# baudm/parseq

Measured on NVIDIA H100. Metric: images/sec PARSeq-S 32x128 AR+1refine, higher is better.
Workload: dtype bf16

## Files before the change

### parseq_b200/build.py

```python
from __future__ import annotations

import os
import shutil
import subprocess

PKG = os.path.dirname(os.path.abspath(__file__))
CSRC = os.path.join(PKG, "csrc")
LIB_DIR = os.path.join(PKG, "lib")
LIB_PATH = os.path.join(LIB_DIR, "libparseq_b200.so")
SOURCES = ["engine.cu"]
HEADERS = ["ptx.cuh", "gemm.cuh", "kernels.cuh", "dec_ar.cuh", "dec_ar2.cuh", "gemm_ln.cuh", "mlp_ln.cuh", "attn_wgmma.cuh", "qkv_attn.cuh", "crops.cuh", os.path.join("..", "..", "include", "parseq_b200.h")]

NVCC_FLAGS = [
    "-gencode", "arch=compute_90a,code=sm_90a", "-lineinfo", "-O3", "-std=c++17",
    "-Xcompiler", "-fPIC", "-shared",
]


def _nvcc() -> str:
    for cand in (os.environ.get("NVCC"), shutil.which("nvcc"), "/usr/local/cuda/bin/nvcc"):
        if cand and os.path.exists(cand):
            return cand
    raise RuntimeError("nvcc not found")


def needs_build() -> bool:
    if not os.path.exists(LIB_PATH):
        return True
    t = os.path.getmtime(LIB_PATH)
    deps = [os.path.join(CSRC, s) for s in SOURCES + HEADERS]
    return any(os.path.getmtime(d) > t for d in deps)


def build(force: bool = False, verbose: bool = False) -> str:
    if not force and not needs_build():
        return LIB_PATH
    import fcntl
    os.makedirs(LIB_DIR, exist_ok=True)
    with open(os.path.join(LIB_DIR, ".build.lock"), "w") as lock:
        fcntl.flock(lock, fcntl.LOCK_EX)
        if not force and not needs_build():
            return LIB_PATH
        tmp = LIB_PATH + f".tmp{os.getpid()}"
        cmd = [_nvcc()] + NVCC_FLAGS + ["-o", tmp] + [os.path.join(CSRC, s) for s in SOURCES]
        if verbose:
            cmd.insert(1, "-Xptxas=-v")
        res = subprocess.run(cmd, capture_output=True, text=True)
        if res.returncode != 0:
            if os.path.exists(tmp):
                os.remove(tmp)
            raise RuntimeError("nvcc failed:\n" + res.stdout + res.stderr)
        os.replace(tmp, LIB_PATH)
        if verbose:
            print(res.stderr)
    return LIB_PATH


if __name__ == "__main__":
    print(build(force=True, verbose=True))
```

### parseq_b200/csrc/engine.cu

```cuda
#include <cuda.h>
#include <cuda_runtime.h>

#include <cmath>
#include <cstdio>
#include <cstdlib>
#include <cstring>
#include <map>
#include <mutex>
#include <set>
#include <string>
#include <type_traits>
#include <vector>

#include "../../include/parseq_b200.h"
#include "gemm.cuh"
#include "kernels.cuh"
#include "dec_ar.cuh"
#include "dec_ar2.cuh"
#include "gemm_ln.cuh"
#include "mlp_ln.cuh"
#include "attn_wgmma.cuh"
#include "qkv_attn.cuh"
#include "crops.cuh"

namespace {

constexpr int kMaxHeadClasses = 16384;
constexpr int kMaxLabelLength = 63;

thread_local std::string g_last_error;

int fail(int code, const std::string& msg) {
  g_last_error = msg;
  return code;
}
#define PQ_CUDA(expr)                                                                              \
  do {                                                                                             \
    cudaError_t _e = (expr);                                                                       \
    if (_e != cudaSuccess)                                                                         \
      return fail(PARSEQ_ERR_CUDA, std::string(#expr) + " -> " + cudaGetErrorString(_e));          \
  } while (0)
#define PQ_TRY(expr)                 \
  do {                               \
    int _r = (expr);                 \
    if (_r != PARSEQ_OK) return _r;  \
  } while (0)

typedef CUresult (*PFN_encodeTiled)(CUtensorMap*, CUtensorMapDataType, cuuint32_t, void*, const cuuint64_t*,
                                    const cuuint64_t*, const cuuint32_t*, const cuuint32_t*, CUtensorMapInterleave,
                                    CUtensorMapSwizzle, CUtensorMapL2promotion, CUtensorMapFloatOOBfill);
PFN_encodeTiled g_encode = nullptr;

int load_driver_api() {
  if (g_encode != nullptr) return PARSEQ_OK;
  void* fn = nullptr;
  cudaDriverEntryPointQueryResult qres;
  cudaError_t e = cudaGetDriverEntryPoint("cuTensorMapEncodeTiled", &fn, cudaEnableDefault, &qres);
  if (e != cudaSuccess || fn == nullptr || qres != cudaDriverEntryPointSuccess)
    return fail(PARSEQ_ERR_CUDA, "cuTensorMapEncodeTiled not available from the driver");
  g_encode = reinterpret_cast<PFN_encodeTiled>(fn);
  return PARSEQ_OK;
}

int make_tmap(CUtensorMap* tm, const void* ptr, int esize, long long rows, long long cols, long long ld, int box_cols,
              int box_rows) {
  PQ_TRY(load_driver_api());
  if ((reinterpret_cast<uintptr_t>(ptr) & 15u) != 0 || ((ld * esize) & 15) != 0)
    return fail(PARSEQ_ERR_INVALID_ARG, "GEMM operand must be 16-byte aligned with a 16-byte multiple row stride");
  cuuint64_t dims[2] = {static_cast<cuuint64_t>(cols), static_cast<cuuint64_t>(rows)};
  cuuint64_t strides[1] = {static_cast<cuuint64_t>(ld) * static_cast<cuuint64_t>(esize)};
  cuuint32_t box[2] = {static_cast<cuuint32_t>(box_cols), static_cast<cuuint32_t>(box_rows)};
  cuuint32_t estr[2] = {1, 1};
  CUresult r = g_encode(tm, esize == 2 ? CU_TENSOR_MAP_DATA_TYPE_BFLOAT16 : CU_TENSOR_MAP_DATA_TYPE_FLOAT32, 2,
// ... 4 lines not shown
  return PARSEQ_OK;
}

int make_tmap3d(CUtensorMap* tm, const void* ptr, long long d0, long long d1, long long d2, long long ld1, long long ld2,
                int box_d0, int box_d1) {
  PQ_TRY(load_driver_api());
  if ((reinterpret_cast<uintptr_t>(ptr) & 15u) != 0 || ((ld1 * 2) & 15) != 0 || ((ld2 * 2) & 15) != 0)
    return fail(PARSEQ_ERR_INVALID_ARG, "tensor map operand must be 16-byte aligned with 16-byte multiple strides");
  cuuint64_t dims[3] = {static_cast<cuuint64_t>(d0), static_cast<cuuint64_t>(d1), static_cast<cuuint64_t>(d2)};
  cuuint64_t strides[2] = {static_cast<cuuint64_t>(ld1) * 2u, static_cast<cuuint64_t>(ld2) * 2u};
  cuuint32_t box[3] = {static_cast<cuuint32_t>(box_d0), static_cast<cuuint32_t>(box_d1), 1u};
  cuuint32_t estr[3] = {1, 1, 1};
  CUresult r = g_encode(tm, CU_TENSOR_MAP_DATA_TYPE_BFLOAT16, 3, const_cast<void*>(ptr), dims, strides, box, estr,
                        CU_TENSOR_MAP_INTERLEAVE_NONE, CU_TENSOR_MAP_SWIZZLE_128B, CU_TENSOR_MAP_L2_PROMOTION_L2_256B,
                        CU_TENSOR_MAP_FLOAT_OOB_FILL_NONE);
  if (r != CUDA_SUCCESS) return fail(PARSEQ_ERR_CUDA, "cuTensorMapEncodeTiled(3d) failed: " + std::to_string(int(r)));
  return PARSEQ_OK;
}

int make_tmap_kv4d(CUtensorMap* tm, const void* ptr, int T, int max_batch, int panels, int box_t) {
  PQ_TRY(load_driver_api());
  if ((reinterpret_cast<uintptr_t>(ptr) & 15u) != 0)
    return fail(PARSEQ_ERR_INVALID_ARG, "tensor map operand must be 16-byte aligned");
  const cuuint64_t row = 128;
  cuuint64_t dims[4] = {64, static_cast<cuuint64_t>(T), static_cast<cuuint64_t>(max_batch), static_cast<cuuint64_t>(panels)};
  cuuint64_t strides[3] = {row, row * T, row * T * max_batch};
  cuuint32_t box[4] = {64, static_cast<cuuint32_t>(box_t), 1u, 1u};
  cuuint32_t estr[4] = {1, 1, 1, 1};
  CUresult r = g_encode(tm, CU_TENSOR_MAP_DATA_TYPE_BFLOAT16, 4, const_cast<void*>(ptr), dims, strides, box, estr,
                        CU_TENSOR_MAP_INTERLEAVE_NONE, CU_TENSOR_MAP_SWIZZLE_128B, CU_TENSOR_MAP_L2_PROMOTION_L2_256B,
                        CU_TENSOR_MAP_FLOAT_OOB_FILL_NONE);
  if (r != CUDA_SUCCESS) return fail(PARSEQ_ERR_CUDA, "cuTensorMapEncodeTiled(K/V 4d) failed: " + std::to_string(int(r)));
  return PARSEQ_OK;
}

uint16_t f32_to_bf16_rne(float f) {
  uint32_t u;
  std::memcpy(&u, &f, 4);
  if ((u & 0x7fffffffu) > 0x7f800000u) return static_cast<uint16_t>((u >> 16) | 0x40u);
  u += 0x7fffu + ((u >> 16) & 1u);
  return static_cast<uint16_t>(u >> 16);
}

struct LaunchOpts {
  int sm_count = 0;
  bool use_pdl = true;
  int ln_cta_group = 0;
  int ln_split = 0;
  int mlp_cta_group = 0;
  bool pair_pdl = false;
  int gemm_stages = 0;
  int attn_impl = 0;
  int ln_clusters = 0;
};
LaunchOpts g_default_opts;

int ensure_sm_count(LaunchOpts& o) {
  if (o.sm_count == 0) {
    int dev = 0;
    PQ_CUDA(cudaGetDevice(&dev));
    PQ_CUDA(cudaDeviceGetAttribute(&o.sm_count, cudaDevAttrMultiProcessorCount, dev));
  }
  return PARSEQ_OK;
}

struct LaunchConfig {
  cudaLaunchConfig_t cfg{};
  cudaLaunchAttribute attr[2];
  LaunchConfig(dim3 grid, dim3 block, size_t smem, cudaStream_t st, unsigned cluster, bool pdl) {
    cfg.gridDim = grid;
    cfg.blockDim = block;
    cfg.dynamicSmemBytes = smem;
    cfg.stream = st;
    cfg.attrs = attr;
    if (cluster > 0) {
      attr[cfg.numAttrs].id = cudaLaunchAttributeClusterDimension;
      attr[cfg.numAttrs].val.clusterDim.x = cluster;
      attr[cfg.numAttrs].val.clusterDim.y = 1;
      attr[cfg.numAttrs].val.clusterDim.z = 1;
      ++cfg.numAttrs;
    }
    if (pdl) {
      attr[cfg.numAttrs].id = cudaLaunchAttributeProgrammaticStreamSerialization;
      attr[cfg.numAttrs].val.programmaticStreamSerializationAllowed = 1;
      ++cfg.numAttrs;
    }
  }
  LaunchConfig(const LaunchConfig&) = delete;
  LaunchConfig& operator=(const LaunchConfig&) = delete;
};

template <typename... KArgs, typename... Args>
int launch_ex(const LaunchConfig& lc, void (*kern)(KArgs...), Args... args) {
  PQ_CUDA(cudaLaunchKernelEx(&lc.cfg, kern, static_cast<KArgs>(args)...));
  return PARSEQ_OK;
}
template <typename... KArgs, typename... Args>
int launch_k(const LaunchOpts& lo, void (*kern)(KArgs...), dim3 grid, dim3 block, size_t smem, cudaStream_t st, Args... args) {
  return launch_ex(LaunchConfig(grid, block, smem, st, 0, lo.use_pdl), kern, args...);
}
bool cluster_pdl(const LaunchOpts& lo, int cg) { return lo.use_pdl && (cg == 1 || lo.pair_pdl); }

template <typename F>
int dispatch_width(int D, const char* what, F&& f) {
  switch (D) {
    case 192: return f(std::integral_constant<int, 192>{});
// ... 42 lines not shown
    else return pq::dec_ar2_kernel<D, MT, CS, HS>;
  }
}
template <typename... KArgs>
int set_smem(void (*kern)(KArgs...), size_t bytes) {
  PQ_CUDA(cudaFuncSetAttribute(kern, cudaFuncAttributeMaxDynamicSharedMemorySize, static_cast<int>(bytes)));
  return PARSEQ_OK;
}
template <int D, int MT, int CS, bool WIDE, int IDP>
int ar2_attr() {
  PQ_TRY(set_smem(ar2_kernel<D, MT, CS, false, WIDE, IDP>(), pq::dec_ar2_smem_bytes<D, MT, CS, IDP>()));
  if constexpr (MT == 1 && CS == 8 && D / 64 <= CS)
    PQ_TRY(set_smem(ar2_kernel<D, MT, CS, true, WIDE, IDP>(), pq::dec_ar2_smem_bytes<D, MT, CS, IDP>()));
  return PARSEQ_OK;
}
template <bool WIDE, int IDP>
int ar2_set_attributes() {
  PQ_TRY((ar2_attr<192, 1, 8, WIDE, IDP>())); PQ_TRY((ar2_attr<192, 2, 8, WIDE, IDP>())); PQ_TRY((ar2_attr<384, 1, 8, WIDE, IDP>()));
  PQ_TRY((ar2_attr<384, 2, 8, WIDE, IDP>())); PQ_TRY((ar2_attr<768, 1, 8, WIDE, IDP>()));
  PQ_TRY((ar2_attr<192, 1, 6, WIDE, IDP>())); PQ_TRY((ar2_attr<192, 2, 6, WIDE, IDP>())); PQ_TRY((ar2_attr<384, 1, 6, WIDE, IDP>()));
  PQ_TRY((ar2_attr<384, 2, 6, WIDE, IDP>())); PQ_TRY((ar2_attr<768, 1, 6, WIDE, IDP>()));
  return PARSEQ_OK;
}

template <int D, int MODE>
int gemm_ln_attr() { return set_smem(pq::gemm_ln_fused_kernel<D, MODE>, pq::GemmLnCfg<D, MODE>::kSmemBytes); }
template <int D, int CG>
int mlp_ln_attr() { return set_smem(pq::mlp_ln_fused_kernel<D, CG>, pq::MlpLnCfg<D, CG>::kSmemBytes); }
template <int NK>
int attn_wgmma_attr() { return set_smem(pq::enc_attention_wgmma_kernel<NK>, pq::atw_smem_bytes<NK>()); }
template <int D>
int qkv_attn_attr() { return set_smem(pq::enc_qkv_attn_kernel<D>, pq::QkvAttnCfg::kSmemBytes); }
template <int EPI, int STORE>
int gemm_attr() { return set_smem(pq::gemm_bf16_wgmma_kernel<EPI, STORE>, pq::GemmCfg::smem_bytes<STORE != pq::ST_REG>()); }
constexpr int kTmaBenchSmem = 12 * pq::A2_SLOT + 1024 + 256;

int init_kernel_attributes() {
  PQ_TRY(set_smem(pq::dec_ar_kernel<192, 1>, pq::dec_ar_smem_bytes<192>()));
  PQ_TRY(set_smem(pq::dec_ar_kernel<192, 2>, pq::dec_ar_smem_bytes<192>()));
  PQ_TRY(set_smem(pq::dec_ar_kernel<384, 1>, pq::dec_ar_smem_bytes<384>()));
  PQ_TRY(set_smem(pq::dec_ar_kernel<384, 2>, pq::dec_ar_smem_bytes<384>()));
  PQ_TRY(set_smem(pq::dec_ar_kernel<768, 1>, pq::dec_ar_smem_bytes<768>()));
  PQ_TRY(set_smem(pq::dec_ar_kernel<768, 2>, pq::dec_ar_smem_bytes<768>()));
  PQ_TRY((ar2_set_attributes<false, 32>()));
  PQ_TRY((ar2_set_attributes<true, 32>()));
  PQ_TRY((ar2_set_attributes<false, 64>()));
  PQ_TRY((ar2_set_attributes<true, 64>()));
  PQ_TRY(set_smem(pq::dec_ln_head_argmax_kernel<192>, 120 * 1024));
  PQ_TRY(set_smem(pq::dec_ln_head_argmax_kernel<384>, 160 * 1024));
  PQ_TRY(set_smem(pq::dec_ln_head_argmax_kernel<768>, 226 * 1024));
  PQ_TRY((gemm_ln_attr<192, 0>())); PQ_TRY((gemm_ln_attr<384, 0>())); PQ_TRY((gemm_ln_attr<192, 1>()));
  PQ_TRY((gemm_ln_attr<384, 1>())); PQ_TRY((gemm_ln_attr<384, 2>()));
  PQ_TRY((mlp_ln_attr<192, 1>())); PQ_TRY((mlp_ln_attr<384, 1>())); PQ_TRY((mlp_ln_attr<192, 2>())); PQ_TRY((mlp_ln_attr<384, 2>()));
  PQ_TRY((attn_wgmma_attr<128>())); PQ_TRY((attn_wgmma_attr<256>()));
  PQ_TRY((qkv_attn_attr<192>())); PQ_TRY((qkv_attn_attr<384>()));
  PQ_TRY((gemm_attr<pq::EPI_F32, pq::ST_REG>()));
  PQ_TRY((gemm_attr<pq::EPI_F32_RESID, pq::ST_REG>()));
  PQ_TRY((gemm_attr<pq::EPI_BF16, pq::ST_REG>()));
  PQ_TRY((gemm_attr<pq::EPI_BF16, pq::ST_TMA_2D>()));
  PQ_TRY((gemm_attr<pq::EPI_BF16, pq::ST_TMA_3D>()));
  PQ_TRY((gemm_attr<pq::EPI_GELU_BF16, pq::ST_REG>()));
  PQ_TRY((gemm_attr<pq::EPI_GELU_BF16, pq::ST_TMA_2D>()));
  PQ_TRY(set_smem(pq::tma_stream_bench_kernel, kTmaBenchSmem));
  int dev = 0, optin = 0;
  PQ_CUDA(cudaGetDevice(&dev));
  PQ_CUDA(cudaDeviceGetAttribute(&optin, cudaDevAttrMaxSharedMemoryPerBlockOptin, dev));
  PQ_TRY(set_smem(pq::crop_resize_bicubic_kernel, static_cast<size_t>(optin)));
  return PARSEQ_OK;
}

int ensure_kernel_attributes() {
  static std::mutex mu;
  static std::set<int> done;
  int dev = 0;
  PQ_CUDA(cudaGetDevice(&dev));
  std::lock_guard<std::mutex> lock(mu);
  if (done.count(dev) != 0) return PARSEQ_OK;
  PQ_TRY(init_kernel_attributes());
  done.insert(dev);
  return PARSEQ_OK;
}

int gemm_launch(LaunchOpts& lo, const void* A, long long lda, const void* W, long long ldw, const float* bias, int M, int N,
                int K, int mode, float alpha, const float* resid, long long ldr, int resid_mod, void* out, long long ldo,
                cudaStream_t st, long long blocked_rows = 0) {
  if (M <= 0 || N <= 0 || K <= 0) return fail(PARSEQ_ERR_INVALID_ARG, "gemm: empty problem");
  if (mode != pq::EPI_F32 && mode != pq::EPI_BF16 && mode != pq::EPI_GELU_BF16)
    return fail(PARSEQ_ERR_INVALID_ARG, "gemm: mode must be 0 (fp32), 1 (bf16) or 2 (GELU bf16)");
  PQ_TRY(ensure_sm_count(lo));
  CUtensorMap ta, tb, to;
  PQ_TRY(make_tmap(&ta, A, 2, M, K, lda, pq::GEMM_BLOCK_K, pq::GEMM_BLOCK_M));
  PQ_TRY(make_tmap(&tb, W, 2, N, K, ldw, pq::GEMM_BLOCK_K, pq::GEMM_BLOCK_N));
  pq::GemmParams p;
  p.M = M; p.N = N; p.K = K; p.alpha = alpha; p.bias = bias;
  p.resid = resid; p.ldr = ldr; p.resid_mod = resid_mod; p.out = out; p.ldo = ldo;
  const int esz = (mode == pq::EPI_F32) ? 4 : 2;
  bool vec = ((reinterpret_cast<uintptr_t>(out) & 7u) == 0) && ((ldo * esz) % 8 == 0);
  if (resid != nullptr) vec = vec && ((reinterpret_cast<uintptr_t>(resid) & 7u) == 0) && ((ldr * 4) % 8 == 0);
  p.vec_ok = vec ? 1 : 0;
  int store = pq::ST_REG;
  if (blocked_rows > 0) {
    if (mode != pq::EPI_BF16 || N % 64 != 0 || blocked_rows < M || (reinterpret_cast<uintptr_t>(out) & 15u) != 0)
      return fail(PARSEQ_ERR_INVALID_ARG, "gemm: blocked output needs a bf16 epilogue, N % 64 == 0 and rows >= M");
    PQ_TRY(make_tmap3d(&to, out, 64, M, N / 64, 64, 64 * blocked_rows, 64, pq::GEMM_BLOCK_M));
    store = pq::ST_TMA_3D;
  } else if (mode != pq::EPI_F32 && (reinterpret_cast<uintptr_t>(out) & 15u) == 0 && (ldo * 2) % 16 == 0 && ldo >= N) {
// ... 31 lines not shown
  pq::GemmLnParams p;
  p.M = M; p.K = K; p.bias = bias; p.gamma = gamma; p.beta = beta; p.eps = eps;
  p.num_m_tiles = (M + Cfg::kTileM - 1) / Cfg::kTileM;
  int clusters = p.num_m_tiles;
  if constexpr (MODE == 2) {
    PQ_TRY(make_tmap(&tx, x, 4, M, D, D, Cfg::kXBoxCols, pq::GLN_BLOCK_M));
    if (lo.ln_clusters == 0) {
      const LaunchConfig occ(dim3(static_cast<unsigned>(lo.sm_count / Cfg::kCG * Cfg::kCG)), dim3(pq::GLN_THREADS),
                             Cfg::kSmemBytes, st, Cfg::kCG, false);
      PQ_CUDA(cudaOccupancyMaxActiveClusters(&lo.ln_clusters, pq::gemm_ln_fused_kernel<D, MODE>, &occ.cfg));
      if (lo.ln_clusters <= 0) return fail(PARSEQ_ERR_CUDA, "gemm_ln: no cluster of the persistent kernel fits the device");
    }
    clusters = std::min(p.num_m_tiles, lo.ln_clusters);
  } else {
    tx = ta;
  }
  return launch_ex(LaunchConfig(dim3(static_cast<unsigned>(clusters * Cfg::kCG)), dim3(pq::GLN_THREADS), Cfg::kSmemBytes, st,
                                Cfg::kCG, cluster_pdl(lo, Cfg::kCG)),
                   pq::gemm_ln_fused_kernel<D, MODE>, ta, tb, tx, x, reinterpret_cast<__nv_bfloat16*>(xn), p);
}
int gemm_ln_launch(LaunchOpts& lo, const void* A, long long lda, const void* W, long long ldw, const float* bias, int M, int D,
                   int K, float* x, const float* gamma, const float* beta, float eps, void* xn, cudaStream_t st) {
  if (M <= 0 || K <= 0) return fail(PARSEQ_ERR_INVALID_ARG, "gemm_ln: empty problem");
  PQ_TRY(ensure_sm_count(lo));
  PQ_TRY(load_driver_api());
  if (D == 384 && lo.ln_split != 1)
    return launch_gemm_ln<384, 2>(lo, A, lda, W, ldw, bias, M, K, x, gamma, beta, eps, xn, st);
  if (lo.ln_cta_group == 2) {
    if (D == 384) return launch_gemm_ln<384, 1>(lo, A, lda, W, ldw, bias, M, K, x, gamma, beta, eps, xn, st);
    if (D == 192) return launch_gemm_ln<192, 1>(lo, A, lda, W, ldw, bias, M, K, x, gamma, beta, eps, xn, st);
  }
  if (D == 384) return launch_gemm_ln<384, 0>(lo, A, lda, W, ldw, bias, M, K, x, gamma, beta, eps, xn, st);
  if (D == 192) return launch_gemm_ln<192, 0>(lo, A, lda, W, ldw, bias, M, K, x, gamma, beta, eps, xn, st);
  return fail(PARSEQ_ERR_UNSUPPORTED, "gemm_ln: embed_dim must be 192 or 384");
}

template <int D, int CG>
int launch_mlp_ln(const LaunchOpts& lo, const void* xn, const void* W1, const float* b1, const void* W2, const float* b2, int M,
                  float* x, const float* gamma, const float* beta, float eps, void* xn_out, cudaStream_t st) {
  using Cfg = pq::MlpLnCfg<D, CG>;
  if ((reinterpret_cast<uintptr_t>(x) & 7u) != 0 || (reinterpret_cast<uintptr_t>(xn_out) & 3u) != 0)
    return fail(PARSEQ_ERR_INVALID_ARG, "mlp_ln: x must be 8-byte and xn_out 4-byte aligned");
  CUtensorMap txn, tw1, tw2;
  PQ_TRY(make_tmap(&txn, xn, 2, M, D, D, 64, pq::GLN_BLOCK_M));
  PQ_TRY(make_tmap(&tw1, W1, 2, Cfg::kH, D, D, 64, Cfg::kW1Rows));
  PQ_TRY(make_tmap(&tw2, W2, 2, D, Cfg::kH, Cfg::kH, 64, Cfg::kW2Rows));
  pq::MlpLnParams p;
  p.M = M; p.b1 = b1; p.b2 = b2; p.gamma = gamma; p.beta = beta; p.eps = eps;
  p.num_m_tiles = (M + pq::GLN_BLOCK_M * CG - 1) / (pq::GLN_BLOCK_M * CG);
  return launch_ex(LaunchConfig(dim3(static_cast<unsigned>(p.num_m_tiles * CG)), dim3(pq::MLP_THREADS), Cfg::kSmemBytes, st, CG,
                                cluster_pdl(lo, CG)),
                   pq::mlp_ln_fused_kernel<D, CG>, txn, tw1, tw2, x, reinterpret_cast<__nv_bfloat16*>(xn_out), p);
}
int mlp_ln_launch(LaunchOpts& lo, const void* xn, const void* W1, const float* b1, const void* W2, const float* b2, int M, int D,
                  float* x, const float* gamma, const float* beta, float eps, void* xn_out, cudaStream_t st) {
  if (M <= 0) return fail(PARSEQ_ERR_INVALID_ARG, "mlp_ln: empty problem");
  PQ_TRY(ensure_sm_count(lo));
  PQ_TRY(load_driver_api());
  const int CG = lo.mlp_cta_group ? lo.mlp_cta_group : 2;
  if (CG == 2) {
    if (D == 384) return launch_mlp_ln<384, 2>(lo, xn, W1, b1, W2, b2, M, x, gamma, beta, eps, xn_out, st);
    if (D == 192) return launch_mlp_ln<192, 2>(lo, xn, W1, b1, W2, b2, M, x, gamma, beta, eps, xn_out, st);
  }
  if (D == 384) return launch_mlp_ln<384, 1>(lo, xn, W1, b1, W2, b2, M, x, gamma, beta, eps, xn_out, st);
  if (D == 192) return launch_mlp_ln<192, 1>(lo, xn, W1, b1, W2, b2, M, x, gamma, beta, eps, xn_out, st);
  return fail(PARSEQ_ERR_UNSUPPORTED, "mlp_ln: embed_dim must be 192 or 384 (hidden width 4 * embed_dim)");
}

int layernorm_launch(const LaunchOpts& lo, const float* x, const float* g, const float* b, float eps, int M, int D, void* y, float* y32,
                     cudaStream_t st, const float* add = nullptr, int add_mod = 1, float* xw = nullptr) {
  const int rows_per_block = 8;
  const int grid = (M + rows_per_block - 1) / rows_per_block;
  __nv_bfloat16* yb = reinterpret_cast<__nv_bfloat16*>(y);
  switch (D) {
    case 192: return launch_k(lo, pq::layernorm_kernel<192>, dim3(grid), dim3(256), 0, st, x, g, b, eps, M, yb, y32, add, add_mod, xw);
    case 384: return launch_k(lo, pq::layernorm_kernel<384>, dim3(grid), dim3(256), 0, st, x, g, b, eps, M, yb, y32, add, add_mod, xw);
    case 768: return launch_k(lo, pq::layernorm_kernel<768>, dim3(grid), dim3(256), 0, st, x, g, b, eps, M, yb, y32, add, add_mod, xw);
    default: return fail(PARSEQ_ERR_UNSUPPORTED, "layernorm: embed_dim must be 192, 384 or 768");
  }
}

int enc_attention_launch(const LaunchOpts& lo, const void* qkv, int B, int T, int D, int heads, void* out, cudaStream_t st) {
  if (D != heads * pq::ATT_DH) return fail(PARSEQ_ERR_UNSUPPORTED, "encoder attention kernels cover head_dim=64");
  if (lo.attn_impl == 1 && T <= 256) {
    const dim3 grid(static_cast<unsigned>(B * heads), static_cast<unsigned>((T + 127) / 128));
    const __nv_bfloat16* q = reinterpret_cast<const __nv_bfloat16*>(qkv);
    __nv_bfloat16* o = reinterpret_cast<__nv_bfloat16*>(out);
    if (T <= 128)
      return launch_k(lo, pq::enc_attention_wgmma_kernel<128>, grid, dim3(pq::ATW_THREADS), pq::atw_smem_bytes<128>(), st, q, o, T, D, heads);
    return launch_k(lo, pq::enc_attention_wgmma_kernel<256>, grid, dim3(pq::ATW_THREADS), pq::atw_smem_bytes<256>(), st, q, o, T, D, heads);
  }
  if (T != pq::ATT_T) {
    return launch_k(lo, pq::enc_attention_any_kernel, dim3(B * heads, (T + pq::ATT_T - 1) / pq::ATT_T), dim3(256), 0, st,
                    reinterpret_cast<const __nv_bfloat16*>(qkv), reinterpret_cast<__nv_bfloat16*>(out), T, D, heads);
  }
  return launch_k(lo, pq::enc_attention_kernel, dim3(B * heads), dim3(256), 0, st,
                  reinterpret_cast<const __nv_bfloat16*>(qkv), reinterpret_cast<__nv_bfloat16*>(out), D, heads);
}

bool qkv_attn_supported(int T, int D, int heads) { return T == pq::ATT_T && D == heads * pq::ATT_DH && (D == 192 || D == 384); }
int qkv_attn_launch(LaunchOpts& lo, const void* xn, const void* W, const float* bias, int B, int T, int D, int heads, void* out,
                    cudaStream_t st) {
  if (B <= 0) return fail(PARSEQ_ERR_INVALID_ARG, "qkv_attn: empty batch");
  if (!qkv_attn_supported(T, D, heads))
    return fail(PARSEQ_ERR_UNSUPPORTED, "qkv_attn: T = 128, head_dim 64 and embed_dim 192 or 384 only");
  if ((reinterpret_cast<uintptr_t>(out) & 15u) != 0) return fail(PARSEQ_ERR_INVALID_ARG, "qkv_attn: out must be 16-byte aligned");
  PQ_TRY(ensure_sm_count(lo));
  CUtensorMap tx, tw;
  PQ_TRY(make_tmap(&tx, xn, 2, static_cast<long long>(B) * T, D, D, pq::GEMM_BLOCK_K, pq::ATT_T));
  PQ_TRY(make_tmap(&tw, W, 2, 3 * D, D, D, pq::GEMM_BLOCK_K, pq::ATT_DH));
  const int items = B * heads;
// ... 1484 lines not shown
  const int D = e->D;
  const int cap = e->dec_chunk * e->L;
  parseq_engine::Stage& sg = e->stages[0];
  for (int r0 = 0; r0 < rows; r0 += cap) {
    const int n = (rows - r0 < cap) ? (rows - r0) : cap;
    const long long n4 = 1ll * n * D / 4;
    pq::f32_to_bf16_kernel<<<static_cast<unsigned>(std::min<long long>((n4 + 255) / 256, 132ll * 8)), 256, 0, e->main>>>(
        reinterpret_cast<const float4*>(x + 1ll * r0 * D), reinterpret_cast<uint2*>(sg.yn), n4);
    PQ_CUDA(cudaGetLastError());
    e->launches++;
    e->cur_cat = CAT_DEC_GEMM;
    PQ_TRY(gemm(e, sg.yn, D, e->w("head.weight"), D, e->wf("head.bias"), n, e->C, D, pq::EPI_F32, 1.0f, nullptr, 0, 0,
                logits + 1ll * r0 * e->C, e->C, e->main));
  }
  PQ_CUDA(cudaEventRecord(e->ev_out, e->main));
  PQ_CUDA(cudaStreamWaitEvent(user, e->ev_out, 0));
  return PARSEQ_OK;
}

int parseq_text_embed(parseq_engine* e, int32_t n, const int32_t* ids, float* out, parseq_stream_t stream) {
  if (e == nullptr || ids == nullptr || out == nullptr) return fail(PARSEQ_ERR_INVALID_ARG, "null argument");
  if (e->arch != 0) return fail(PARSEQ_ERR_UNSUPPORTED, "text_embed: PARSeq only");
  if (n <= 0) return n == 0 ? PARSEQ_OK : fail(PARSEQ_ERR_INVALID_ARG, "negative count");
  if (!e->slots[e->index.at("text_embed.embedding.weight")].set) return fail(PARSEQ_ERR_STATE, "weights not set");
  PQ_CUDA(cudaSetDevice(e->cfg.device));
  const long long total = 1ll * n * e->D;
  pq::text_embed_kernel<<<static_cast<unsigned>(std::min<long long>((total + 255) / 256, 132ll * 8)), 256, 0,
                          reinterpret_cast<cudaStream_t>(stream)>>>(ids, e->wf("text_embed.embedding.weight"), out, n, e->D, e->V,
                                                                    std::sqrt(static_cast<float>(e->D)));
  PQ_CUDA(cudaGetLastError());
  return PARSEQ_OK;
}

int parseq_bench_tma_stream(void* buf, int64_t bytes, int cluster, int ctas, int nboxes, int nslot, int mode, void* sink,
                            parseq_stream_t stream) {
  if (buf == nullptr || sink == nullptr || cluster < 1 || cluster > 8 || ctas % cluster != 0 || nslot < 1 || nslot > 12)
    return fail(PARSEQ_ERR_INVALID_ARG, "bench_tma_stream: bad arguments");
  const long long rows_total = 8192;
  const int blocks = static_cast<int>(bytes / (rows_total * 128));
  if (blocks < 1) return fail(PARSEQ_ERR_INVALID_ARG, "bench_tma_stream: buffer too small");
  PQ_TRY(ensure_kernel_attributes());
  CUtensorMap map;
  PQ_TRY(make_tmap3d(&map, buf, 64, rows_total, blocks, 64, 64 * rows_total, 64, 128));
  return launch_ex(LaunchConfig(dim3(static_cast<unsigned>(ctas)), dim3(pq::A2_THREADS + 32), kTmaBenchSmem,
                                reinterpret_cast<cudaStream_t>(stream), cluster > 1 ? static_cast<unsigned>(cluster) : 0, false),
                   pq::tma_stream_bench_kernel, map, nboxes, nslot, static_cast<int>(rows_total / 128), blocks, mode,
                   static_cast<unsigned int*>(sink));
}

int64_t parseq_debug_int(parseq_engine* e, const char* name) {
  if (name == nullptr) return -1;
  const std::string n(name);
  if (n == "ln_clusters") return (e ? e->lo : g_default_opts).ln_clusters;
  if (e == nullptr) return -1;
  if (n == "ar2_occupancy_mt1_cs8") return e->ar2_occ[1][0];
  if (n == "ar2_occupancy_mt2_cs8") return e->ar2_occ[2][0];
  if (n == "ar2_occupancy_mt1_cs6") return e->ar2_occ[1][1];
  if (n == "ar2_occupancy_mt2_cs6") return e->ar2_occ[2][1];
  if (n == "ar_last_cluster_size") return e->ar_last_cs;
  if (n == "ar_last_per") return e->ar_last_per;
  if (n == "ar_last_clusters") return e->ar_last_ncl;
  if (n == "ar_last_mt") return e->ar_last_mt;
  if (n == "ar_last_head_split") return e->ar_last_hs;
  if (n == "ar_last_wide") return e->ar_last_wide;
  if (n == "ar_last_ids_pitch") return e->ar_last_idp;
  if (n == "sm_count") return e->lo.sm_count;
  return -1;
}
int64_t parseq_kernel_launches(const parseq_engine* e) { return e ? e->launches : 0; }

int parseq_set_option(parseq_engine* e, const char* name, int64_t value) {
  if (name == nullptr) return fail(PARSEQ_ERR_INVALID_ARG, "null option");
  const std::string n(name);
  LaunchOpts& lo = e ? e->lo : g_default_opts;
  if (n == "block_n") {
    if (value != 0 && value != 64 && value != 128 && value != 192 && value != 256)
      return fail(PARSEQ_ERR_INVALID_ARG, "block_n: 0/64/128/192/256");
    return PARSEQ_OK;
  }
  if (n == "cta_group") {
    if (value < 0 || value > 2) return fail(PARSEQ_ERR_INVALID_ARG, "cta_group: 0 (auto) / 1 / 2");
    return PARSEQ_OK;
  }
  if (n == "attn_impl") { lo.attn_impl = value != 0 ? 1 : 0; if (e) drop_graphs(e); return PARSEQ_OK; }
  if (n == "pdl") { lo.use_pdl = value != 0; if (e) drop_graphs(e); return PARSEQ_OK; }
  if (n == "gemm_stages") {
    if (value < 0 || value == 1) return fail(PARSEQ_ERR_INVALID_ARG, "gemm_stages: 0 (full ring) or >= 2");
    lo.gemm_stages = static_cast<int>(value);
    if (e) drop_graphs(e);
    return PARSEQ_OK;
  }
  if (n == "ln_cta_group") {
    if (value < 0 || value > 2) return fail(PARSEQ_ERR_INVALID_ARG, "ln_cta_group: 0 (auto) / 1 / 2");
    lo.ln_cta_group = static_cast<int>(value);
    if (e) drop_graphs(e);
    return PARSEQ_OK;
  }
  if (n == "ln_split") {
    if (value < 0 || value > 2) return fail(PARSEQ_ERR_INVALID_ARG, "ln_split: 0 (auto) / 1 (off) / 2 (on)");
    lo.ln_split = static_cast<int>(value);
    if (e) drop_graphs(e);
    return PARSEQ_OK;
  }
  if (n == "mlp_cta_group") {
    if (value < 0 || value > 2) return fail(PARSEQ_ERR_INVALID_ARG, "mlp_cta_group: 0 (auto) / 1 / 2");
    lo.mlp_cta_group = static_cast<int>(value);
// ... 134 lines not shown
```

### parseq_b200/csrc/ptx.cuh

```cuda
#pragma once
#include <cuda_bf16.h>
#include <cuda_runtime.h>
#include <stdint.h>

namespace pq {

__device__ __forceinline__ uint32_t smem_u32(const void* p) {
  return static_cast<uint32_t>(__cvta_generic_to_shared(p));
}
__device__ __forceinline__ uint32_t lane_id() { return threadIdx.x & 31u; }

constexpr int ARGMAX_NONE = 0x7fffffff;
__device__ __forceinline__ bool argmax_better(float v, int j, float best, int bi) {
  if (j == ARGMAX_NONE) return false;
  if (bi == ARGMAX_NONE) return true;
  const bool vn = isnan(v), bn = isnan(best);
  if (vn != bn) return vn;
  if (vn || v == best) return j < bi;
  return v > best;
}
__device__ __forceinline__ void argmax_fold(float& best, int& bi, float v, int j) {
  if (argmax_better(v, j, best, bi)) { best = v; bi = j; }
}
__device__ __forceinline__ void argmax_shfl(float& best, int& bi, int lo = 1, int hi = 32) {
// ... 103 lines not shown
__device__ __forceinline__ void prefetch_tmap(const void* tmap) {
  asm volatile("prefetch.tensormap [%0];" ::"l"(reinterpret_cast<uint64_t>(tmap)) : "memory");
}
__device__ __forceinline__ void tma_load_2d(void* smem_dst, const void* tmap, uint64_t* bar, int32_t c0,
                                            int32_t c1) {
  asm volatile(
      "cp.async.bulk.tensor.2d.shared::cluster.global.mbarrier::complete_tx::bytes [%0], [%1, {%3, %4}], [%2];"
      ::"r"(smem_u32(smem_dst)), "l"(reinterpret_cast<uint64_t>(tmap)), "r"(smem_u32(bar)), "r"(c0), "r"(c1)
      : "memory");
}

__device__ __forceinline__ void tma_load_3d(void* smem_dst, const void* tmap, uint64_t* bar, int32_t c0, int32_t c1,
                                            int32_t c2) {
  asm volatile(
      "cp.async.bulk.tensor.3d.shared::cluster.global.mbarrier::complete_tx::bytes [%0], [%1, {%3, %4, %5}], [%2];"
      ::"r"(smem_u32(smem_dst)), "l"(reinterpret_cast<uint64_t>(tmap)), "r"(smem_u32(bar)), "r"(c0), "r"(c1), "r"(c2)
      : "memory");
}

__device__ __forceinline__ void tma_load_4d(void* smem_dst, const void* tmap, uint64_t* bar, int32_t c0, int32_t c1,
                                            int32_t c2, int32_t c3) {
  asm volatile(
      "cp.async.bulk.tensor.4d.shared::cluster.global.mbarrier::complete_tx::bytes [%0], [%1, {%3, %4, %5, %6}], [%2];"
      ::"r"(smem_u32(smem_dst)), "l"(reinterpret_cast<uint64_t>(tmap)), "r"(smem_u32(bar)), "r"(c0), "r"(c1), "r"(c2),
        "r"(c3)
      : "memory");
}

__device__ __forceinline__ void tma_store_2d(const void* tmap, const void* smem_src, int32_t c0, int32_t c1) {
  asm volatile("cp.async.bulk.tensor.2d.global.shared::cta.bulk_group [%0, {%2, %3}], [%1];"
               ::"l"(reinterpret_cast<uint64_t>(tmap)), "r"(smem_u32(smem_src)), "r"(c0), "r"(c1)
               : "memory");
}
__device__ __forceinline__ void tma_store_3d(const void* tmap, const void* smem_src, int32_t c0, int32_t c1, int32_t c2) {
  asm volatile("cp.async.bulk.tensor.3d.global.shared::cta.bulk_group [%0, {%2, %3, %4}], [%1];"
               ::"l"(reinterpret_cast<uint64_t>(tmap)), "r"(smem_u32(smem_src)), "r"(c0), "r"(c1), "r"(c2)
               : "memory");
}
__device__ __forceinline__ void tma_reduce_add_2d(const void* tmap, const void* smem_src, int32_t c0, int32_t c1) {
  asm volatile("cp.reduce.async.bulk.tensor.2d.global.shared::cta.add.tile.bulk_group [%0, {%2, %3}], [%1];"
               ::"l"(reinterpret_cast<uint64_t>(tmap)), "r"(smem_u32(smem_src)), "r"(c0), "r"(c1)
               : "memory");
}
__device__ __forceinline__ void bulk_commit_group() { asm volatile("cp.async.bulk.commit_group;" ::: "memory"); }
template <int N>
__device__ __forceinline__ void bulk_wait_group_read() {
  asm volatile("cp.async.bulk.wait_group.read %0;" ::"n"(N) : "memory");
}
template <int N>
__device__ __forceinline__ void bulk_wait_group() {
  asm volatile("cp.async.bulk.wait_group %0;" ::"n"(N) : "memory");
}
__device__ __forceinline__ void fence_proxy_async_smem() { asm volatile("fence.proxy.async.shared::cta;" ::: "memory"); }

__device__ __forceinline__ void tma_load_2d_mcast(void* smem_dst, const void* tmap, uint64_t* bar, int32_t c0, int32_t c1,
                                                  uint16_t cta_mask) {
  asm volatile(
      "cp.async.bulk.tensor.2d.shared::cluster.global.mbarrier::complete_tx::bytes.multicast::cluster [%0], [%1, {%3, %4}], [%2], %5;"
      ::"r"(smem_u32(smem_dst)), "l"(reinterpret_cast<uint64_t>(tmap)), "r"(smem_u32(bar)), "r"(c0), "r"(c1), "h"(cta_mask)
      : "memory");
}
__device__ __forceinline__ void mbar_wait_cluster(uint64_t* bar, uint32_t parity) {
  uint32_t ok = 0;
  long long t0 = clock64();
  uint32_t it = 0;
  while (true) {
    asm volatile(
        "{\n\t.reg .pred p;\n\t"
        "mbarrier.try_wait.parity.acquire.cluster.shared::cta.b64 p, [%1], %2;\n\t"
        "selp.b32 %0, 1, 0, p;\n\t}"
        : "=r"(ok)
        : "r"(smem_u32(bar)), "r"(parity)
        : "memory");
    if (ok) return;
    if (((++it) & 0x3ffu) == 0 && (clock64() - t0) > PQ_SPIN_LIMIT_CYCLES) __trap();
  }
}
__device__ __forceinline__ void st_cluster_f32(uint32_t cluster_addr, float v) {
  asm volatile("st.shared::cluster.f32 [%0], %1;" ::"r"(cluster_addr), "f"(v) : "memory");
}

__device__ __forceinline__ uint64_t make_desc_k_sw128(uint32_t smem_addr) {
  uint64_t d = 0;
  d |= static_cast<uint64_t>((smem_addr >> 4) & 0x3FFFu);
  d |= static_cast<uint64_t>(1u) << 16;
  d |= static_cast<uint64_t>(1024u >> 4) << 32;
  d |= static_cast<uint64_t>(1u) << 62;
  return d;
}
__device__ __forceinline__ void wgmma_fence() { asm volatile("wgmma.fence.sync.aligned;" ::: "memory"); }
__device__ __forceinline__ void wgmma_commit() { asm volatile("wgmma.commit_group.sync.aligned;" ::: "memory"); }
template <int N>
__device__ __forceinline__ void wgmma_wait() { asm volatile("wgmma.wait_group.sync.aligned %0;" ::"n"(N) : "memory"); }
template <int R>
__device__ __forceinline__ void wgmma_reg_fence(float (&d)[R]) {
#pragma unroll
  for (int i = 0; i < R; ++i) asm volatile("" : "+f"(d[i])::"memory");
}

template <int N>
__device__ __forceinline__ void wgmma_bf16(float (&d)[N / 2], uint64_t da, uint64_t db, uint32_t accumulate);
template <>
__device__ __forceinline__ void wgmma_bf16<32>(float (&d)[16], uint64_t da, uint64_t db, uint32_t accumulate) {
  asm volatile(
      "{\n\t.reg .pred p;\n\tsetp.ne.b32 p, %18, 0;\n\t"
      "wgmma.mma_async.sync.aligned.m64n32k16.f32.bf16.bf16 {%0, %1, %2, %3, %4, %5, %6, %7, %8, %9, %10, %11, %12, %13, %14, %15}, %16, %17, p, 1, 1, 0, 0;\n\t}"
// ... 99 lines not shown
```

Before: 41390.

## Add persistent CTA-pair fused MLP+LayerNorm kernel for D=384

Adds a persistent, warp-specialized MLP+residual+LayerNorm kernel for D=384 that splits the hidden and output columns across a 2-CTA cluster. Each CTA computes half of every fc1 chunk and sends its GELU slice to the peer through DSMEM bulk copies, then accumulates half the fc2 output columns. Two consumer warpgroups each handle a 64-row tile. The aim is to cut per-CTA weight traffic and register pressure and to get steady pipelining across M tiles. The cost is cross-CTA synchronization on every chunk plus extra complexity. It becomes the default path for D=384.

```diff
diff --git a/parseq_b200/build.py b/parseq_b200/build.py
--- a/parseq_b200/build.py
+++ b/parseq_b200/build.py
@@ -9,7 +9,7 @@
 LIB_DIR = os.path.join(PKG, "lib")
 LIB_PATH = os.path.join(LIB_DIR, "libparseq_b200.so")
 SOURCES = ["engine.cu"]
-HEADERS = ["ptx.cuh", "gemm.cuh", "kernels.cuh", "dec_ar.cuh", "dec_ar2.cuh", "gemm_ln.cuh", "mlp_ln.cuh", "attn_wgmma.cuh", "qkv_attn.cuh", "crops.cuh", os.path.join("..", "..", "include", "parseq_b200.h")]
+HEADERS = ["ptx.cuh", "gemm.cuh", "kernels.cuh", "dec_ar.cuh", "dec_ar2.cuh", "gemm_ln.cuh", "mlp_ln.cuh", "mlp_ln_pair.cuh", "attn_wgmma.cuh", "qkv_attn.cuh", "crops.cuh", os.path.join("..", "..", "include", "parseq_b200.h")]
 
 NVCC_FLAGS = [
     "-gencode", "arch=compute_90a,code=sm_90a", "-lineinfo", "-O3", "-std=c++17",
diff --git a/parseq_b200/csrc/engine.cu b/parseq_b200/csrc/engine.cu
--- a/parseq_b200/csrc/engine.cu
+++ b/parseq_b200/csrc/engine.cu
@@ -19,6 +19,7 @@
 #include "dec_ar2.cuh"
 #include "gemm_ln.cuh"
 #include "mlp_ln.cuh"
+#include "mlp_ln_pair.cuh"
 #include "attn_wgmma.cuh"
 #include "qkv_attn.cuh"
 #include "crops.cuh"
@@ -129,6 +130,7 @@
   int gemm_stages = 0;
   int attn_impl = 0;
   int ln_clusters = 0;
+  int mlp_clusters = 0;
 };
 LaunchOpts g_default_opts;
 
@@ -277,6 +279,7 @@
   PQ_TRY((gemm_ln_attr<192, 0>())); PQ_TRY((gemm_ln_attr<384, 0>())); PQ_TRY((gemm_ln_attr<192, 1>()));
   PQ_TRY((gemm_ln_attr<384, 1>())); PQ_TRY((gemm_ln_attr<384, 2>()));
   PQ_TRY((mlp_ln_attr<192, 1>())); PQ_TRY((mlp_ln_attr<384, 1>())); PQ_TRY((mlp_ln_attr<192, 2>())); PQ_TRY((mlp_ln_attr<384, 2>()));
+  PQ_TRY(set_smem(pq::mlp_ln_pair_kernel, pq::MlpLnPairCfg::kSmemBytes));
   PQ_TRY((attn_wgmma_attr<128>())); PQ_TRY((attn_wgmma_attr<256>()));
   PQ_TRY((qkv_attn_attr<192>())); PQ_TRY((qkv_attn_attr<384>()));
   PQ_TRY((gemm_attr<pq::EPI_F32, pq::ST_REG>()));
@@ -414,11 +417,36 @@
                                 cluster_pdl(lo, CG)),
                    pq::mlp_ln_fused_kernel<D, CG>, txn, tw1, tw2, x, reinterpret_cast<__nv_bfloat16*>(xn_out), p);
 }
+int launch_mlp_ln_pair(LaunchOpts& lo, const void* xn, const void* W1, const float* b1, const void* W2, const float* b2, int M,
+                       float* x, const float* gamma, const float* beta, float eps, void* xn_out, cudaStream_t st) {
+  using Cfg = pq::MlpLnPairCfg;
+  constexpr int D = Cfg::kD;
+  if ((reinterpret_cast<uintptr_t>(xn_out) & 3u) != 0) return fail(PARSEQ_ERR_INVALID_ARG, "mlp_ln: xn_out must be 4-byte aligned");
+  CUtensorMap txn, tw1, tw2, tx;
+  PQ_TRY(make_tmap(&txn, xn, 2, M, D, D, 64, pq::GLN_BLOCK_M));
+  PQ_TRY(make_tmap(&tw1, W1, 2, Cfg::kH, D, D, 64, 64));
+  PQ_TRY(make_tmap(&tw2, W2, 2, D, Cfg::kH, Cfg::kH, 64, Cfg::kCols));
+  PQ_TRY(make_tmap(&tx, x, 4, M, D, D, pq::GemmLnCfg<D, 2>::kXBoxCols, pq::GLN_BLOCK_M));
+  pq::MlpLnParams p;
+  p.M = M; p.b1 = b1; p.b2 = b2; p.gamma = gamma; p.beta = beta; p.eps = eps;
+  p.num_m_tiles = (M + Cfg::kUnitM - 1) / Cfg::kUnitM;
+  if (lo.mlp_clusters == 0) {
+    const LaunchConfig occ(dim3(static_cast<unsigned>(lo.sm_count / Cfg::kCG * Cfg::kCG)), dim3(pq::MLP_THREADS), Cfg::kSmemBytes,
+                           st, Cfg::kCG, false);
+    PQ_CUDA(cudaOccupancyMaxActiveClusters(&lo.mlp_clusters, pq::mlp_ln_pair_kernel, &occ.cfg));
+    if (lo.mlp_clusters <= 0) return fail(PARSEQ_ERR_CUDA, "mlp_ln: no cluster of the persistent kernel fits the device");
+  }
+  const int clusters = std::min(p.num_m_tiles, lo.mlp_clusters);
+  return launch_ex(LaunchConfig(dim3(static_cast<unsigned>(clusters * Cfg::kCG)), dim3(pq::MLP_THREADS), Cfg::kSmemBytes, st,
+                                Cfg::kCG, cluster_pdl(lo, Cfg::kCG)),
+                   pq::mlp_ln_pair_kernel, txn, tw1, tw2, tx, x, reinterpret_cast<__nv_bfloat16*>(xn_out), p);
+}
 int mlp_ln_launch(LaunchOpts& lo, const void* xn, const void* W1, const float* b1, const void* W2, const float* b2, int M, int D,
                   float* x, const float* gamma, const float* beta, float eps, void* xn_out, cudaStream_t st) {
   if (M <= 0) return fail(PARSEQ_ERR_INVALID_ARG, "mlp_ln: empty problem");
   PQ_TRY(ensure_sm_count(lo));
   PQ_TRY(load_driver_api());
+  if (D == 384 && lo.mlp_cta_group == 0) return launch_mlp_ln_pair(lo, xn, W1, b1, W2, b2, M, x, gamma, beta, eps, xn_out, st);
   const int CG = lo.mlp_cta_group ? lo.mlp_cta_group : 2;
   if (CG == 2) {
     if (D == 384) return launch_mlp_ln<384, 2>(lo, xn, W1, b1, W2, b2, M, x, gamma, beta, eps, xn_out, st);
@@ -2009,6 +2037,7 @@
   if (name == nullptr) return -1;
   const std::string n(name);
   if (n == "ln_clusters") return (e ? e->lo : g_default_opts).ln_clusters;
+  if (n == "mlp_clusters") return (e ? e->lo : g_default_opts).mlp_clusters;
   if (e == nullptr) return -1;
   if (n == "ar2_occupancy_mt1_cs8") return e->ar2_occ[1][0];
   if (n == "ar2_occupancy_mt2_cs8") return e->ar2_occ[2][0];
diff --git a/parseq_b200/csrc/mlp_ln_pair.cuh b/parseq_b200/csrc/mlp_ln_pair.cuh
--- /dev/null
+++ b/parseq_b200/csrc/mlp_ln_pair.cuh
@@ -0,0 +1,251 @@
+#pragma once
+#include "mlp_ln.cuh"
+
+namespace pq {
+
+struct MlpLnPairCfg {
+  static constexpr int kD = 384;
+  static constexpr int kH = 4 * kD;
+  static constexpr int kCG = 2;
+  static constexpr int kUnitM = 2 * GLN_BLOCK_M;
+  static constexpr int kChunks = kH / 128;
+  static constexpr int kCols = kD / 2;
+  static constexpr int kKB1 = kD / 64;
+  static constexpr int kW1KBytes = 64 * 64 * 2;
+  static constexpr int kStageBytes = kCols * 64 * 2;
+  static constexpr int kStages = 3;
+  static constexpr int kActBytes = GLN_BLOCK_M * kD * 2;
+  static constexpr int kHidKBBytes = GLN_BLOCK_M * 64 * 2;
+  static constexpr int kHidBytes = 2 * kHidKBBytes;
+  static constexpr int kParamBytes = (kChunks * 64 + 3 * kCols) * 4 + 2 * 2 * 4 * GLN_BLOCK_M * 4;
+  static constexpr int kBarBytes = 256;
+  static constexpr int kSmemBytes = kStages * kStageBytes + 2 * kActBytes + 2 * kHidBytes + kParamBytes + kBarBytes + 1024;
+  static_assert(kStageBytes == 3 * kW1KBytes && kKB1 == 6, "an fc1 chunk is two stages");
+  static_assert(kActBytes == GemmLnCfg<kD, 2>::kXBytes, "the x slice of gln_pair_epilogue fits the xn tile's buffer");
+  static_assert(kCols <= 256, "one W2 box");
+  static_assert(kSmemBytes <= 232448, "shared memory");
+};
+
+__global__ void __launch_bounds__(MLP_THREADS, 1)
+mlp_ln_pair_kernel(const __grid_constant__ CUtensorMap tmXn, const __grid_constant__ CUtensorMap tmW1,
+                   const __grid_constant__ CUtensorMap tmW2, const __grid_constant__ CUtensorMap tmX,
+                   float* __restrict__ x, __nv_bfloat16* __restrict__ xn_out, const MlpLnParams p) {
+  using Cfg = MlpLnPairCfg;
+  constexpr int D = Cfg::kD;
+  extern __shared__ uint8_t smem_raw[];
+  const uint32_t raw_addr = smem_u32(smem_raw);
+  const uint32_t pad = ((raw_addr + 1023u) & ~1023u) - raw_addr;
+  uint8_t* ring = smem_raw + pad;
+  uint8_t* act = ring + Cfg::kStages * Cfg::kStageBytes;
+  uint8_t* hid = act + 2 * Cfg::kActBytes;
+  float* s_b1 = reinterpret_cast<float*>(hid + 2 * Cfg::kHidBytes);
+  float* s_b2 = s_b1 + Cfg::kChunks * 64;
+  float* s_gamma = s_b2 + Cfg::kCols;
+  float* s_beta = s_gamma + Cfg::kCols;
+  float* s_part = s_beta + Cfg::kCols;
+  uint64_t* full_bar = reinterpret_cast<uint64_t*>(reinterpret_cast<uint8_t*>(s_b1) + Cfg::kParamBytes);
+  uint64_t* empty_bar = full_bar + Cfg::kStages;
+  uint64_t* act_full = empty_bar + Cfg::kStages;
+  uint64_t* act_empty = act_full + 2;
+  uint64_t* hid_full = act_empty + 2;
+  uint64_t* hid_empty = hid_full + 2;
+  uint64_t* stat_bar = hid_empty + 2;
+
+  const uint32_t rank = cluster_ctarank();
+  const uint32_t peer = rank ^ 1u;
+  const int r = static_cast<int>(rank & 1u);
+  const int c0 = r * Cfg::kCols;
+  const int cluster = static_cast<int>(blockIdx.x / Cfg::kCG), clusters = static_cast<int>(gridDim.x / Cfg::kCG);
+
+  grid_dep_launch();
+  if (threadIdx.x == 0) {
+    prefetch_tmap(&tmXn);
+    prefetch_tmap(&tmW1);
+    prefetch_tmap(&tmW2);
+    prefetch_tmap(&tmX);
+    for (int s = 0; s < Cfg::kStages; ++s) {
+      mbar_init(&full_bar[s], 1);
+      mbar_init(&empty_bar[s], 2);
+    }
+    for (int w = 0; w < 2; ++w) {
+      mbar_init(&act_full[w], 1);
+      mbar_init(&act_empty[w], 128);
+      mbar_init(&hid_full[w], 1);
+      mbar_init(&hid_empty[w], 1);
+    }
+    for (int i = 0; i < 4; ++i) mbar_init(&stat_bar[i], 2 * 128);
+    fence_mbar_init();
+  }
+  for (int j = threadIdx.x; j < Cfg::kChunks * 64; j += MLP_THREADS)
+    s_b1[j] = __ldg(p.b1 + (2 * (j >> 6) + r) * 64 + (j & 63));
+  for (int j = threadIdx.x; j < Cfg::kCols; j += MLP_THREADS) {
+    s_b2[j] = __ldg(p.b2 + c0 + j);
+    s_gamma[j] = __ldg(p.gamma + c0 + j);
+    s_beta[j] = __ldg(p.beta + c0 + j);
+  }
+  cluster_sync_all();
+  grid_dep_wait();
+
+  if (threadIdx.x < 128) {
+    setmaxnreg_dec<40>();
+    if (threadIdx.x == 0) {
+      int stage = 0;
+      uint32_t phase = 0;
+      auto next = [&]() -> uint8_t* {
+        mbar_wait_mma(&empty_bar[stage], phase ^ 1u);
+        mbar_expect_tx(&full_bar[stage], Cfg::kStageBytes);
+        return ring + stage * Cfg::kStageBytes;
+      };
+      auto advance = [&]() { if (++stage == Cfg::kStages) { stage = 0; phase ^= 1u; } };
+      auto load_w1 = [&](int c, int half) {
+        uint8_t* dst = next();
+#pragma unroll
+        for (int i = 0; i < 3; ++i)
+          tma_load_2d(dst + i * Cfg::kW1KBytes, &tmW1, &full_bar[stage], (3 * half + i) * 64, (2 * c + r) * 64);
+        advance();
+      };
+      auto load_w2 = [&](int kb) {
+        tma_load_2d(next(), &tmW2, &full_bar[stage], kb * 64, c0);
+        advance();
+      };
+      for (int u = cluster; u < p.num_m_tiles; u += clusters) {
+        for (int c = 0; c < Cfg::kChunks; ++c) {
+          load_w1(c, 0);
+          load_w1(c, 1);
+          load_w2(2 * c);
+          load_w2(2 * c + 1);
+        }
+      }
+    } else if (threadIdx.x == 32) {
+      uint32_t f = 0;
+      for (int u = cluster; u < p.num_m_tiles; u += clusters) {
+        for (int w = 0; w < 2; ++w) {
+          mbar_wait_mma(&act_empty[w], (f & 1u) ^ 1u);
+          mbar_expect_tx(&act_full[w], Cfg::kActBytes);
+#pragma unroll
+          for (int b = 0; b < Cfg::kKB1; ++b)
+            tma_load_2d(act + w * Cfg::kActBytes + b * Cfg::kW1KBytes, &tmXn, &act_full[w], b * 64, (2 * u + w) * GLN_BLOCK_M);
+        }
+        ++f;
+        for (int w = 0; w < 2; ++w) {
+          mbar_wait_mma(&act_empty[w], (f & 1u) ^ 1u);
+          mbar_expect_tx(&act_full[w], Cfg::kActBytes);
+#pragma unroll
+          for (int b = 0; b < Cfg::kCols / GemmLnCfg<D, 2>::kXBoxCols; ++b)
+            tma_load_2d(act + w * Cfg::kActBytes + b * GemmLnCfg<D, 2>::kXBoxBytes, &tmX, &act_full[w],
+                        c0 + b * GemmLnCfg<D, 2>::kXBoxCols, (2 * u + w) * GLN_BLOCK_M);
+        }
+        ++f;
+      }
+    }
+    __syncwarp();
+  } else {
+    setmaxnreg_inc<232>();
+    const int wg = (threadIdx.x >> 7) - 1;
+    const int t = threadIdx.x & 127;
+    const int lane = t & 31;
+    const bool leader = t == 0;
+    const uint32_t act_addr = smem_u32(act + wg * Cfg::kActBytes);
+    uint8_t* own_kb = hid + wg * Cfg::kHidBytes + r * Cfg::kHidKBBytes;
+    const uint32_t hid_addr = smem_u32(hid + wg * Cfg::kHidBytes);
+    const uint32_t peer_kb = mapa_cluster(smem_u32(own_kb), peer);
+    const uint32_t peer_hid_full = mapa_cluster(smem_u32(&hid_full[wg]), peer);
+    const uint32_t peer_hid_empty = mapa_cluster(smem_u32(&hid_empty[wg]), peer);
+    int stage = 0, prev = -1;
+    uint32_t phase = 0, par = 0;
+    uint32_t n = 0;
+
+    auto retire = [&]() {
+      wgmma_wait<1>();
+      if (prev >= 0 && leader) mbar_arrive(&empty_bar[prev]);
+      prev = stage;
+      if (++stage == Cfg::kStages) { stage = 0; phase ^= 1u; }
+    };
+    auto drain = [&]() {
+      wgmma_wait<0>();
+      if (prev >= 0 && leader) mbar_arrive(&empty_bar[prev]);
+      prev = -1;
+    };
+    auto fc1_stage = [&](float (&h)[32], int half) {
+      mbar_wait_mma(&full_bar[stage], phase);
+      const uint32_t base = smem_u32(ring + stage * Cfg::kStageBytes);
+      wgmma_fence();
+#pragma unroll
+      for (int i = 0; i < 3; ++i) {
+        const int kk = 3 * half + i;
+        const uint64_t da = make_desc_k_sw128(act_addr + kk * Cfg::kW1KBytes);
+        const uint64_t db = make_desc_k_sw128(base + i * Cfg::kW1KBytes);
+#pragma unroll
+        for (int k = 0; k < 4; ++k)
+          wgmma_bf16<64>(h, da + static_cast<uint64_t>(2 * k), db + static_cast<uint64_t>(2 * k), static_cast<uint32_t>((kk | k) != 0));
+      }
+      wgmma_commit();
+      retire();
+    };
+    float acc[Cfg::kCols / 2];
+#pragma unroll
+    for (int i = 0; i < Cfg::kCols / 2; ++i) acc[i] = 0.0f;
+    auto fc2_stage = [&](int kb) {
+      mbar_wait_mma(&full_bar[stage], phase);
+      const uint64_t da = make_desc_k_sw128(hid_addr + (kb & 1) * Cfg::kHidKBBytes);
+      const uint64_t db = make_desc_k_sw128(smem_u32(ring + stage * Cfg::kStageBytes));
+      wgmma_fence();
+#pragma unroll
+      for (int k = 0; k < 4; ++k)
+        wgmma_bf16<Cfg::kCols>(acc, da + static_cast<uint64_t>(2 * k), db + static_cast<uint64_t>(2 * k), static_cast<uint32_t>((kb | k) != 0));
+      wgmma_commit();
+      retire();
+    };
+    float h[32];
+#pragma unroll 1
+    for (int u = cluster; u < p.num_m_tiles; u += clusters) {
+      const int m0 = (2 * u + wg) * GLN_BLOCK_M;
+      mbar_wait_mma(&act_full[wg], 0);
+      fc1_stage(h, 0);
+      fc1_stage(h, 1);
+#pragma unroll 1
+      for (int c = 0; c < Cfg::kChunks; ++c) {
+        drain();
+        if (c > 0 && leader) mbar_arrive_cluster(peer_hid_empty);
+        if (c + 1 == Cfg::kChunks) mbar_arrive(&act_empty[wg]);
+        wgmma_reg_fence(h);
+        if (n > 0) mbar_wait_cluster(&hid_empty[wg], (n - 1) & 1u);
+#pragma unroll
+        for (int i = 0; i < 8; ++i) {
+          const int col = i * 8 + 2 * (lane & 3);
+          const float b0 = s_b1[c * 64 + col], b1 = s_b1[c * 64 + col + 1];
+#pragma unroll
+          for (int hr = 0; hr < 2; ++hr) {
+            const int row = (t >> 5) * 16 + (lane >> 2) + hr * 8;
+            *reinterpret_cast<uint32_t*>(own_kb + row * 128 + ((i ^ (lane >> 2)) << 4) + (lane & 3) * 4) =
+                pack_bf16(gelu_erf(h[4 * i + 2 * hr] + b0), gelu_erf(h[4 * i + 2 * hr + 1] + b1));
+          }
+        }
+        fence_proxy_async_smem();
+        named_bar_sync(1 + wg, 128);
+        if (leader) {
+          bulk_copy_to_cluster(peer_kb, own_kb, Cfg::kHidKBBytes, peer_hid_full);
+          mbar_expect_tx(&hid_full[wg], Cfg::kHidKBBytes);
+        }
+        mbar_wait_cluster(&hid_full[wg], n & 1u);
+        fc2_stage(2 * c);
+        fc2_stage(2 * c + 1);
+        ++n;
+        if (c + 1 < Cfg::kChunks) {
+          fc1_stage(h, 0);
+          fc1_stage(h, 1);
+        }
+      }
+      drain();
+      if (leader) mbar_arrive_cluster(peer_hid_empty);
+      wgmma_reg_fence(acc);
+      mbar_wait_mma(&act_full[wg], 1);
+      gln_pair_epilogue<D, 4>(acc, act + wg * Cfg::kActBytes, x, xn_out, p.M, p.eps, m0, c0, rank, s_b2, s_gamma, s_beta,
+                              s_part + wg * 2 * 4 * GLN_BLOCK_M, stat_bar + 2 * wg, par, &act_empty[wg]);
+      par ^= 1u;
+    }
+  }
+  cluster_sync_all();
+}
+
+}
diff --git a/parseq_b200/csrc/ptx.cuh b/parseq_b200/csrc/ptx.cuh
--- a/parseq_b200/csrc/ptx.cuh
+++ b/parseq_b200/csrc/ptx.cuh
@@ -179,6 +179,11 @@
   asm volatile("cp.async.bulk.wait_group %0;" ::"n"(N) : "memory");
 }
 __device__ __forceinline__ void fence_proxy_async_smem() { asm volatile("fence.proxy.async.shared::cta;" ::: "memory"); }
+__device__ __forceinline__ void bulk_copy_to_cluster(uint32_t dst_cluster, const void* src, uint32_t bytes, uint32_t bar_cluster) {
+  asm volatile("cp.async.bulk.shared::cluster.shared::cta.mbarrier::complete_tx::bytes [%0], [%1], %2, [%3];"
+               ::"r"(dst_cluster), "r"(smem_u32(src)), "r"(bytes), "r"(bar_cluster)
+               : "memory");
+}
 
 __device__ __forceinline__ void tma_load_2d_mcast(void* smem_dst, const void* tmap, uint64_t* bar, int32_t c0, int32_t c1,
                                                   uint16_t cta_mask) {
```

After: 41430, median of 6. No clear change (+0.1%).
